# createamind/Distributed-DRL

Hardware: AMD Instinct MI355X
Metric: env-steps/s + learner updates/s, SAC1 LunarLanderContinuous-v2 @1/2/4/8 GPU (higher is better)
Workload: dtype f32

## Files before the change

### distributed-drl_amd/csrc/sac1.hip

```cpp
#include "gemm_core.h"
#include "policy_row.h"

namespace {
struct L1Job {
    const float *in0, *in1, *W, *b;
    float *out, *aug_out;
    int d0, d1, rows, h1, ldo, aug_ld;
    int pre_only;
};
constexpr int MAX_L1_JOBS = 8;
struct OptState;
struct L1Jobs {
    int njobs;
    int noise_on, act, n_each;
    uint32_t noise_seed;
    float *e0, *e1, *e2;
    const OptState *opt;
    L1Job job[MAX_L1_JOBS];
};

constexpr int L1_ROWS = 16;
constexpr int L1_MAXD = 40;
using ddrl_pol::normal_at;
using ddrl_pol::PolRow;
// ... 715 lines not shown
    DDRL_REQUIRE(c->hidden1 <= 64 * RV && c->hidden2 <= 64 * RV, "hidden sizes > 512 unsupported by the row kernels");
    return DDRL_OK;
}

static bool direct_ok(const ddrl_sac1_config_t &c) {
    return c.hidden1 % 4 == 0 && c.hidden2 % 4 == 0 && c.hidden1 <= 512 && c.hidden2 <= 32 * DNT &&
           c.obs_dim + c.act_dim <= 12 && 2 * c.act_dim <= DFH && c.act_dim <= 4 && c.batch <= 4 * DGMAX * 8 &&
           getenv("DDRL_SAC1_GENERIC") == nullptr;
}

}

struct LaunchState {
    int opt_cur;
    int sh_cur;
    bool fuse_apply;
    bool sample_armed;
    bool noise_armed;
    uint32_t noise_seed;
    unsigned int noise_pending;
    bool grad_imported;
};

struct ddrl_sac1 {
    int device;
    ddrl_sac1_config_t cfg;
    Layout L;
    float *slab;
    float *main_p, *target_p, *m, *v, *grad;
    float *in[2][8];
    float *H1, *H2, *dZ2, *dZ1, *xa, *xp, *part;
    float *act0, *act2, *logp0, *logp1, *save0, *q1o, *q2o, *dq4, *dhead, *loss_part, *losses;
    int ldh1, ldh2, ldxa, ldxp, ldd;
    OptState *opt;
    LaunchState ls;
    Seg *segs_d;
    L1Jobs l1a[2];
    GemmJobs g_fa, g_fb, g_bq, g_bpi, g_last;
    RowsA ra[2];
    RowsB rb[2];
    RowsC rc;
    RowsAV rav[2];
    RowsBV rbv[2];
    float *vo, *vto;
    AdamArgs ad;
    int rows_b_blocks;
    bool fused;
    DFHead fh_a[2], fh_b[2];
    DFArgs f_a[2], f_b[2];
    DGJobs dg_bq[2], dg_mid, dg_pi;
    int bq_cols;
    DGJob bq_rest;
    int Lp1, Lp2;
    float *H1r4, *H2c4, *H2r4, *dZ1r4, *dzpi_c4, *dzpi_r4, *dhead_r4, *xa_r4, *da_part, *dq, *w3snap, *xp_r4;
    float *c4_pi[2], *c4_q[3];
    float *c4_q2b;
    int mid_rest_job;
    int bq_q2_job;
    int mid_pi_job, mid_q2w_job;
    int pi_w2_job;
    float *xv_r4;
    int *part_cnt;
    ddrl_replay_dev::RingState *smp_rs;
    ddrl_replay_dev::RingPtrs smp_ring;
    int smp_set;
    float *hp;
    bool fused_l1_wgrad;
    struct HostGraph { const float *block; float *losses; uint32_t seed; int opt_cur, sh_cur; hipGraphExec_t exec; };
    std::vector<HostGraph> host_graphs;
    uint32_t *host_ctr_d;
    struct { bool valid; LaunchState ls; } snap;
};

static void refresh_shadows(ddrl_sac1 *h, hipStream_t s);
int ddrl_internal_normal_fill_ctr(float *out_d, int64_t n, uint32_t seed, const uint32_t *ctr_d, uint64_t base, void *stream);
int ddrl_internal_host_block_up(const float *src, float *dst_d, int64_t n, float *e0, float *e1, float *e2, int64_t m, uint32_t seed,
                                const uint32_t *ctr, void *stream);

static int sac1_free(ddrl_sac1 *h) {
    for (auto &g : h->host_graphs) (void)hipGraphExecDestroy(g.exec);
    if (h->host_ctr_d) (void)hipFree(h->host_ctr_d);
    (void)hipFree(h->slab);
    delete h;
    return DDRL_OK;
}

static int reset_opt(ddrl_sac1 *h, hipStream_t s) {
    OptState o{};
    o.b1p_pi = o.b1p_q = (float)h->cfg.beta1;
    o.b2p_pi = o.b2p_q = (float)h->cfg.beta2;
    h->ls.opt_cur = 0;
    DDRL_HIP_CHECK(hipMemcpyAsync(h->opt, &o, sizeof(o), hipMemcpyHostToDevice, s));
    DDRL_HIP_CHECK(hipStreamSynchronize(s));
    return DDRL_OK;
}

enum { NET_PI = 0, NET_Q1, NET_Q2, NET_V };
enum { ACT_NONE = 0, ACT_STORED, ACT_PI };

struct Eval {
    int net;
    bool x2, targ;
    int act;
    int img = -1;
    bool r4 = false;
    float *ddrl_sac1::*xr4 = nullptr;
    int pev = -1, side = 0;
// ... 216 lines not shown
            dg_add(Q, j);
        }
        for (int q = 0; q < V.nv; ++q) {
            const ValueNet &vn = V.vn[q];
            DGJob j = dq_job(vn.slot, vn.img, q, h->dZ1r4 + q * H1I);
            j.gw_snap = h->w3snap + 512 * q;
            if (vn.net != NET_Q2) { dg_add(Q, j); continue; }
            if (split) j.N = keep * 32;
            h->bq_q2_job = Q.njobs;
            dg_add(Q, j);
            if (split && st == 0) {
                const long long noff = (long long)keep * 32 * 4;
                DGJob r = dq_job(vn.slot, vn.img, q, h->dZ1r4 + q * H1I + noff);
                r.N = h1 - keep * 32;
                r.B = h->c4_q[q] + noff;
                r.mask = h->H1r4 + vn.img * H1I + noff;
                h->bq_rest = r;
            }
        }
    }
    float *G = h->grad;
    const AdamCtx ctx{0, h->main_p, h->target_p, h->m, h->v, G, h->opt, nullptr, L.n_pi_int,
                      (float)cfg->lr, (float)cfg->beta1, (float)cfg->beta2, (float)cfg->adam_eps,
                      (float)cfg->polyak, (float)(1.0 - cfg->polyak), 0u};
    auto wgrad_j4 = [&](const float *A, const float *Bm, long long w_off, long long b_off, float *shadow) {
        DGJob j{};
        j.type = DG_WGRAD_J4; j.M = h1 + 1; j.N = h2; j.K = B;
        j.A = A; j.lda = h->Lp1; j.B = Bm; j.ldb = h->Lp2;
        j.adam_off = w_off; j.ldc = Np2; j.bias_off = b_off; j.bias_row = h1; j.shadow = shadow; j.ld_sh = Kp1;
        return j;
    };
    auto wgrad_rm = [&](const float *A, int lda, int M, const float *Bm, int ldb, int N, long long off) {
        DGJob j{};
        j.type = DG_WGRAD_RM; j.M = M; j.N = N; j.K = B; j.A = A; j.lda = lda; j.B = Bm; j.ldb = ldb; j.adam_off = off; j.ldc = N;
        return j;
    };
    auto head_wgrad = [&](int q) {
        return wgrad_rm(h->H2r4 + V.vn[q].net * H2R, h->Lp2, h2 + 1, h->dq + (long long)q * B, 1, 1, net_off(L, V.vn[q].net).W3);
    };
    {
        DGJobs &M = h->dg_mid;
        M = DGJobs{};
        M.B = B; M.Bv = Bv; M.ad = ctx;
        DGJob d{};
        d.type = DG_DGRAD; d.M = B; d.N = h1; d.K = h2; d.A = h->H2c4; d.lda = B; d.B = h->c4_pi[0]; d.ldb = Kp1;
        d.bgen = 3; d.dap = h->da_part; d.nparts = ct; d.save0 = h->save0; d.wmu = Pm + L.pi_Wmu; d.wls = Pm + L.pi_Wls;
        d.nact = a; d.alpha = (float)cfg->alpha; d.scale = (float)cfg->act_scale;
        d.mask = h->H1r4; d.ldmask = h->Lp1; d.C = h->dZ1r4 + V.nv * H1I; d.ldc = h->Lp1; d.adam_off = -1;
        h->mid_pi_job = M.njobs;
        dg_add(M, d);
        DGJob rc{};
        rc.type = DG_ROWS_C; rc.M = B; rc.N = h2; rc.K = 0; rc.nact = a; rc.adam_off = -1;
        rc.h2c4 = h->H2c4; rc.dap = h->da_part; rc.nparts = ct; rc.save0 = h->save0;
        rc.wmu = Pm + L.pi_Wmu; rc.wls = Pm + L.pi_Wls; rc.dz_c4 = h->dzpi_c4; rc.dz_r4 = h->dzpi_r4; rc.dhead_r4 = h->dhead_r4;
        rc.ld_r4 = h->Lp2; rc.alpha = (float)cfg->alpha; rc.scale = (float)cfg->act_scale;
        dg_add(M, rc);
        for (int q = 0; q < V.nv; ++q) {
            const ValueNet &vn = V.vn[q];
            const NetOff n = net_off(L, vn.net);
            DGJob j = wgrad_j4(h->H1r4 + vn.img * H1I, h->H2r4 + vn.net * H2R, n.W2, n.b2, h->c4_q[q]);
            j.bgen = 1; j.gw = h->w3snap + 512 * q; j.gdq = h->dq + (long long)q * B;
            if (vn.net == NET_Q2) h->mid_q2w_job = M.njobs;
            dg_add(M, j);
        }
        h->mid_rest_job = -1;
        if (!split) {
            for (int q = 0; q < V.nv; ++q) dg_add(M, head_wgrad(q));
        } else {
            const DGJobs &Q0 = h->dg_bq[0];
            M.hp = Q0.hp; M.sacv = 0; M.q_ev0 = Q0.q_ev0; M.q_nev = Q0.q_nev;
            M.b3q1 = Q0.b3q1; M.b3q2 = Q0.b3q2; M.b3q1t = Q0.b3q1t; M.b3q2t = Q0.b3q2t;
            M.rew = Q0.rew; M.done = Q0.done; M.logp0 = Q0.logp0; M.logp1 = Q0.logp1;
            M.q1o = Q0.q1o; M.q2o = Q0.q2o; M.dq = Q0.dq; M.loss_part = Q0.loss_part;
            M.alpha = Q0.alpha; M.gamma = Q0.gamma;
            h->mid_rest_job = M.njobs;
            dg_add(M, h->bq_rest);
        }
    }
    {
        DGJobs &P = h->dg_pi;
        P = DGJobs{};
        P.B = B; P.Bv = Bv; P.ad = ctx;
        h->pi_w2_job = P.njobs;
        dg_add(P, wgrad_j4(h->H1r4, h->dzpi_r4, L.pi_W2, L.pi_b2, h->c4_pi[1]));
        dg_add(P, wgrad_rm(h->H2r4, h->Lp2, h2 + 1, h->dhead_r4, 32, a, L.pi_Wmu));
        dg_add(P, wgrad_rm(h->H2r4, h->Lp2, h2 + 1, h->dhead_r4 + (long long)a * 4, 32, a, L.pi_Wls));
        for (int q = 0; q <= V.nv; ++q) {
            const int net = q < V.nv ? V.vn[q].net : NET_PI;
            const bool xa = net == NET_Q1 || net == NET_Q2;
            DGJob j = wgrad_rm(xa ? h->xa_r4 : (net == NET_V ? h->xv_r4 : h->xp_r4), 32, (xa ? o + a : o) + 1, h->dZ1r4 + q * H1I, h->Lp1, h1, net_off(L, net).W1);
            j.type = DG_WGRAD_W1Y;
            dg_add(P, j);
        }
        if (split)
            for (int q = 0; q < V.nv; ++q) dg_add(P, head_wgrad(q));
        DGJob ls{};
        ls.type = DG_LOSS; ls.M = 1; ls.N = 1; ls.K = 0; ls.adam_off = -1; ls.loss_part = h->loss_part; ls.losses = h->losses; ls.nl = V.nl;
        ls.nparts = -1;
        dg_add(P, ls);
    }
    return DDRL_OK;
}

static void build_rows(ddrl_sac1 *h) {
    const Variant &V = variant_of(h);
    const ddrl_sac1_config_t *cfg = &h->cfg;
    const Layout &L = h->L;
// ... 10 lines not shown
                                (float)cfg->act_scale};
            h->rbv[st] = RowsBV{h->H2, net_q(Pm, L, 0), net_q(Pm, L, 1), net_v(Pm, L), in[3], in[4], h->logp0, h->q1o, h->q2o,
                                h->vo, h->vto, h->dZ2, h->dq4, h->loss_part, B, h2, ldh2, (float)cfg->alpha, (float)cfg->gamma};
        } else {
            h->ra[st] = RowsA{h->H2, net_pi(Pm, L), net_pi(Pt, L), net_q(Pm, L, 0), net_q(Pm, L, 1), in[5], in[6], in[7],
                              h->act0, h->act2, h->logp0, h->logp1, h->save0, h->q1o, h->q2o,
                              h->H1, Pm + L.q_W1[0] + (long long)o * h1, Pt + L.q_W1[0] + (long long)o * h1,
                              Pt + L.q_W1[1] + (long long)o * h1, B, h2, ldh2, a, h1, ldh1, (float)cfg->act_scale};
            h->rb[st] = RowsB{h->H2, net_q(Pm, L, 0), net_q(Pm, L, 1), net_q(Pt, L, 0), net_q(Pt, L, 1), in[3], in[4],
                              h->logp0, h->logp1, h->q1o, h->q2o, h->dZ2, h->dq4, h->loss_part, B, h2, ldh2,
                              (float)cfg->alpha, (float)cfg->gamma};
        }
    }
    h->rc = RowsC{h->H2, at(h->dZ1, 2 * BZ1), Pm + L.q_W1[0], net_pi(Pm, L), h->save0, h->dhead, at(h->dZ2, (V.nv + 1) * BZ2),
                  h->loss_part, h->losses, B, h1, h2, ldh2, o, a, h->ldd, h->rows_b_blocks, (float)cfg->alpha,
                  (float)cfg->act_scale, V.nl};
}

static void init_shape(ddrl_sac1 *h) {
    const ddrl_sac1_config_t &c = h->cfg;
    h->fused = direct_ok(c);
    h->L = make_layout(c, false, h->fused);
    h->Lp1 = rup32(c.hidden1 + 1); h->Lp2 = rup32(c.hidden2 + 1);
    h->ldh1 = (int)pad4(c.hidden1 + 1); h->ldh2 = (int)pad4(c.hidden2 + 1);
    h->ldxa = (int)pad4(c.obs_dim + c.act_dim + 1); h->ldxp = (int)pad4(c.obs_dim + 1); h->ldd = (int)pad4(2 * c.act_dim);
    h->rows_b_blocks = rows_of(h);
    h->mid_rest_job = -1;
}

struct SlabPlan {
    struct Item { float **p; size_t off; };
    std::vector<Item> items;
    size_t floats = 0, cnt_off = 0, opt_off = 0, segs_off = 0;
    size_t reserve(size_t cnt) { const size_t off = floats; floats += (cnt + 63) & ~(size_t)63; return off; }
    void add(float *&p, size_t cnt) { items.push_back(Item{&p, reserve(cnt)}); }
};
static SlabPlan plan_slab(ddrl_sac1 *h) {
    const ddrl_sac1_config_t &c = h->cfg;
    const size_t B = (size_t)rows_of(h), o = c.obs_dim, a = c.act_dim, h1 = c.hidden1, h2 = c.hidden2;
    const size_t NT = (size_t)h->L.total_int, Kp1 = h->L.Kp1, Np2 = h->L.Np2, Lp1 = h->Lp1, Lp2 = h->Lp2;
    SlabPlan p;
    p.add(h->main_p, NT); p.add(h->target_p, NT); p.add(h->m, NT); p.add(h->v, NT); p.add(h->grad, NT);
    for (int st = 0; st < 2; ++st) {
        const size_t cnt[8] = {B * o, B * o, B * a, B, B, B * a, B * a, B * a};
        for (int i = 0; i < 8; ++i) p.add(h->in[st][i], cnt[i]);
    }
    p.add(h->part, ((B + 31) / 32) * (o + 1) * h1);
    if (!h->fused) {
        p.add(h->H1, NEVAL * B * h->ldh1); p.add(h->H2, NEVAL * B * h->ldh2);
        p.add(h->dZ2, 5 * B * h2); p.add(h->dZ1, 5 * B * h1);
    } else {
        const size_t xv = c.variant == DDRL_SAC_V ? 1 : 0;
        p.add(h->H1r4, (4 + xv) * B * Lp1); p.add(h->H2c4, (4 + xv) * Np2 * B); p.add(h->H2r4, (3 + xv) * B * Lp2);
        p.add(h->dZ1r4, (3 + xv) * B * Lp1) ; p.add(h->dzpi_c4, Np2 * B); p.add(h->dzpi_r4, B * Lp2);
        p.add(h->dhead_r4, B * 32); p.add(h->xa_r4, B * 32); p.add(h->xv_r4, B * 32); p.add(h->xp_r4, B * 32); p.add(h->da_part, 16 * B * 4);
        p.add(h->dq, 3 * B + 256); p.add(h->w3snap, 3 * 512);
        for (int i = 0; i < 2; ++i) p.add(h->c4_pi[i], Np2 * Kp1);
        for (size_t i = 0; i < 2 + xv; ++i) p.add(h->c4_q[i], Np2 * Kp1);
        p.add(h->c4_q2b, Np2 * Kp1);
    }
    p.add(h->xa, B * h->ldxa); p.add(h->xp, B * h->ldxp);
    p.add(h->act0, B * a); p.add(h->act2, B * a); p.add(h->logp0, B); p.add(h->logp1, B); p.add(h->save0, B * a * 4);
    p.add(h->q1o, B); p.add(h->q2o, B); p.add(h->vo, B); p.add(h->vto, B); p.add(h->dq4, 3 * B * 4); p.add(h->dhead, B * h->ldd);
    p.add(h->loss_part, (size_t)h->rows_b_blocks * 4); p.add(h->losses, 4);
    p.add(h->hp, (size_t)NEVAL * DFH * B * DNT);
    p.cnt_off = p.reserve(64);
    p.opt_off = p.reserve((2 * sizeof(OptState) + 3) / 4);
    p.segs_off = p.reserve((h->L.segs.size() * sizeof(Seg) + 3) / 4);
    (void)p.reserve(2048);
    return p;
}
static void bind_slab(ddrl_sac1 *h, const SlabPlan &p, float *base) {
    h->slab = base;
    for (const auto &it : p.items) *it.p = base + it.off;
    h->opt = reinterpret_cast<OptState *>(base + p.opt_off);
    h->part_cnt = reinterpret_cast<int *>(base + p.cnt_off);
    h->segs_d = reinterpret_cast<Seg *>(base + p.segs_off);
}
static int alloc_slab(ddrl_sac1 *h, const SlabPlan &p) {
    float *base = nullptr;
    hipError_t e = hipMalloc((void **)&base, p.floats * sizeof(float));
    if (e == hipSuccess) e = hipMemset(base, 0, p.floats * sizeof(float));
    if (e != hipSuccess) {
        ddrl::set_error("hipMalloc of %zu bytes failed in ddrl_sac1_create: %s", p.floats * sizeof(float), hipGetErrorString(e));
        if (base) (void)hipFree(base);
        return DDRL_ERR_NOMEM;
    }
    bind_slab(h, p, base);
    DDRL_HIP_CHECK(hipMemcpy(h->segs_d, h->L.segs.data(), h->L.segs.size() * sizeof(Seg), hipMemcpyHostToDevice));
    return reset_opt(h, nullptr);
}

static int fill_ones(ddrl_sac1 *h) {
    const ddrl_sac1_config_t &c = h->cfg;
    const int B = rows_of(h), o = c.obs_dim, a = c.act_dim, h1 = c.hidden1, h2 = c.hidden2;
    if (!h->fused) {
        k_fill_col<<<(NEVAL * B + 255) / 256, 256>>>(h->H1, (long long)NEVAL * B, h->ldh1, h1, 1.0f);
        k_fill_col<<<(NEVAL * B + 255) / 256, 256>>>(h->H2, (long long)NEVAL * B, h->ldh2, h2, 1.0f);
    } else {
        const int xv = c.variant == DDRL_SAC_V ? 1 : 0;
        k_fill_col4<<<((4 + xv) * B / 4 + 255) / 256, 256>>>(h->H1r4, (long long)(4 + xv) * B / 4, h->Lp1, h1);
        k_fill_col4<<<((3 + xv) * B / 4 + 255) / 256, 256>>>(h->H2r4, (long long)(3 + xv) * B / 4, h->Lp2, h2);
        k_fill_col4<<<(B / 4 + 255) / 256, 256>>>(h->xa_r4, (long long)B / 4, 32, o + a);
        k_fill_col4<<<(B / 4 + 255) / 256, 256>>>(h->xv_r4, (long long)B / 4, 32, o);
        k_fill_col4<<<(B / 4 + 255) / 256, 256>>>(h->xp_r4, (long long)B / 4, 32, o);
    }
    k_fill_col<<<(B + 255) / 256, 256>>>(h->xa, B, h->ldxa, o + a, 1.0f);
// ... 1147 lines not shown
```

### distributed-drl_amd/csrc/sac1_direct.h

```cpp

#ifdef DDRL_STAMPS
static unsigned long long *g_st_host = nullptr;
#define DST(kid, i) do { if (st_ && threadIdx.x == 0) st_[((kid) * 1024 + blockIdx.x) * 16 + (i)] = __builtin_amdgcn_s_memtime(); } while (0)
#define DRT(kid, i) do { if (st_ && threadIdx.x == 0) st_[((kid) * 1024 + blockIdx.x) * 16 + (i)] = __builtin_amdgcn_s_memrealtime(); } while (0)
#else
#define DST(kid, i) do { } while (0)
#define DRT(kid, i) do { } while (0)
#endif

constexpr int DFH = 8;
constexpr int DNT = 16;
constexpr int DGMAX = 16;

__device__ __forceinline__ float f4e(const float4 &v, int e) { return e == 0 ? v.x : (e == 1 ? v.y : (e == 2 ? v.z : v.w)); }

__device__ __forceinline__ void st_img(float *p, const float4 &v) {
    typedef float f4v __attribute__((ext_vector_type(4)));
    f4v t = {v.x, v.y, v.z, v.w};
    __builtin_nontemporal_store(t, reinterpret_cast<f4v *>(p));
}
__device__ __forceinline__ void st_dg(float *p, const float4 &v) {
    typedef float f4v __attribute__((ext_vector_type(4)));
    f4v t = {v.x, v.y, v.z, v.w};
    asm volatile("global_store_dwordx4 %0, %1, off sc1" ::"v"(p), "v"(t) : "memory");
}
__device__ __forceinline__ void st_opt(float *p, const float4 &v) { *reinterpret_cast<float4 *>(p) = v; }
__device__ __forceinline__ int d_slot(int s, int h) { return s < 4 ? 4 * h + s : 8 + 2 * (s - 4) + h; }
__device__ __forceinline__ float relu1(float x) {
    float y;
    asm("v_max_f32 %0, 0, %1" : "=v"(y) : "v"(x));
    return y;
}
static inline int rup32(int x) { return (x + 31) & ~31; }

template <int BYTES>
__device__ __forceinline__ int kline(const void *rec) {
    const int *q = reinterpret_cast<const int *>(rec);
    int acc = q[(BYTES - 4) / 4];
#pragma unroll
    for (int o = 0; o < BYTES - 4; o += 64) acc |= q[o / 4];
    return acc;
}
__device__ __forceinline__ void ktouch(int v) { asm volatile("" ::"s"(v)); }
__device__ __forceinline__ float zero_here() {
    float z = 0.f;
    asm volatile("" : "+v"(z));
    return z;
}

struct DFJob {
    const float *b2;
    const float *wh0, *wh1;
    int nh, hsplit, hstride;
    float *hp;
    float *H2c4;
    float *H2r4;
    float *H1r4;
    float *aug;
    float *xr4;
    int aug_ld;
    const float *php;
    int side;
};
struct DFArgs {
    int njobs, tiles_n, act, Lp1, Lp2, h2;
    float scale;
    float *act0, *act2, *logp0, *logp1, *save0;
    const float *php1;
#ifdef DDRL_STAMPS
    unsigned long long *st;
#endif
    int pev_pack;
    int pin_pack;
    int noise_on, n_each;
    int Bv;
    uint32_t noise_seed;
    float *e0, *e1, *e2;
    const OptState *opt;
    int do_sample, sample_batch;
    ddrl_replay_dev::RingState *rs;
    ddrl_replay_dev::RingPtrs ring;
    ddrl_replay_dev::BatchPtrs sout;
    DFJob job[5];
};
struct DFHead {
    const float *base;
    int tpj, tiles_m;
    int K, Np;
    int B, d0;
    int main_off, targ_off;
    int npi, perq;
    int hp_off;
    int x_off;
    int pack;
};

__host__ __device__ __forceinline__ int pi_bmu_off(int K, int Np, int h2, int act) {
    const int Kp = (K + 31) & ~31;
    return Kp * 16 + Kp * Np + Np + h2 * act;
}
__host__ __device__ __forceinline__ int pi_bls_off(int K, int Np, int h2, int act) { return ((pi_bmu_off(K, Np, h2, act) + act + 3) & ~3) + h2 * act; }

#ifndef DDRL_SIDE_SPREAD
#define DDRL_SIDE_SPREAD 3
#endif
__host__ __device__ __forceinline__ int side_aug_tile(int tiles_n) { return (DDRL_SIDE_SPREAD & 2) ? tiles_n - 1 : 0; }
__host__ __device__ __forceinline__ int side_noise_tile(int tiles_n) { return (DDRL_SIDE_SPREAD & 2) ? (tiles_n > 2 ? tiles_n - 2 : tiles_n - 1) : 0; }
__host__ __device__ __forceinline__ int h1_owned(int b0, int nb, int nt, int tiles_n) {
    if (!(DDRL_SIDE_SPREAD & 1)) return nt == 0 ? 15 : 0;
    int r = b0 % tiles_n, m = 0;
#pragma unroll
    for (int bi = 0; bi < 4; ++bi) {
        if (bi < nb && r == nt) m |= 1 << bi;
        r = r + 1 == tiles_n ? 0 : r + 1;
    }
    return m;
}

template <int NS>
__device__ __forceinline__ void dblock(const float (&w1)[8], const float (&xin)[7], const float4 (&bq)[4], int nrq, floatx16 &x1, floatx16 &acc) {
#pragma unroll
    for (int r = 0; r < 16; ++r) x1[r] = 0.f;
#pragma unroll
    for (int s = 0; s < NS; ++s) x1 = __builtin_amdgcn_mfma_f32_32x32x2f32(w1[s], xin[s], x1, 0, 0, 0);
#pragma unroll
    for (int r = 0; r < 16; ++r) x1[r] = relu1(x1[r]);
#pragma unroll
    for (int rq = 0; rq < 4; ++rq) {
        if (rq < nrq) {
            acc = __builtin_amdgcn_mfma_f32_32x32x2f32(x1[4 * rq + 0], bq[rq].x, acc, 0, 0, 0);
            acc = __builtin_amdgcn_mfma_f32_32x32x2f32(x1[4 * rq + 1], bq[rq].y, acc, 0, 0, 0);
            acc = __builtin_amdgcn_mfma_f32_32x32x2f32(x1[4 * rq + 2], bq[rq].z, acc, 0, 0, 0);
            acc = __builtin_amdgcn_mfma_f32_32x32x2f32(x1[4 * rq + 3], bq[rq].w, acc, 0, 0, 0);
        }
    }
}

struct DOps {
    float4 bq[4][4];
    float w1[4][8];
};
#ifndef DDRL_DPRE0
#define DDRL_DPRE0 1
#endif
#ifndef DDRL_DPRE1
#define DDRL_DPRE1 1
#endif
constexpr int DPRE = 1;
#ifndef DDRL_DGP0
#define DDRL_DGP0 2
#endif
#ifndef DDRL_DGMID
#define DDRL_DGMID 4
#endif
constexpr int DGP0 = DDRL_DGP0;
constexpr int DGMID = DDRL_DGMID;
#ifndef DDRL_DGST
#define DDRL_DGST 5
// ... 208 lines not shown
                ev[c] = pep[0][c];
            }
            const PolRow o = policy_row(mu, ls, ev, d1, a.scale);
    #pragma unroll
            for (int s = 0; s < 7; ++s) {
                const int d = d_slot(s, h), c = d - d0;
                if (d >= d0 && d < D) xin[0][s] = c == 0 ? o.act[0] : (c == 1 ? o.act[1] : (c == 2 ? o.act[2] : o.act[3]));
            }
            if (first_n && w == 0 && lane < 32) {
                const int row = m0 + l31;
                if (jb.side == 1) {
                    a.logp0[row] = o.logp;
    #pragma unroll
                    for (int c = 0; c < 4; ++c)
                        if (c < d1) {
                            a.act0[row * d1 + c] = o.act[c];
                            *reinterpret_cast<float4 *>(a.save0 + ((long long)row * d1 + c) * 4) = make_float4(o.a[c], o.std[c], o.t[c], ev[c]);
                        }
                } else if (jb.side == 2) {
    #pragma unroll
                    for (int c = 0; c < 4; ++c)
                        if (c < d1) a.act2[row * d1 + c] = o.act[c];
                }
            }
            if (two && w == 1) {
    #pragma unroll
                for (int c = 0; c < 4; ++c) {
                    const float o2 = __shfl_xor(hs[1][c], 32);
                    mu[c] = (h ? o2 : hs[1][c]) + pbm[1][c];
                    ls[c] = (h ? hs[1][c] : o2) + pbl[1][c];
                    ev[c] = pep[1][c];
                }
                const PolRow o1 = policy_row(mu, ls, ev, d1, a.scale);
                if (lane < 32) a.logp1[m0 + l31] = o1.logp;
            }
        }
        DST(PH, 2);
        floatx16 acc[MT];
    #pragma unroll
        for (int tt = 0; tt < MT; ++tt)
    #pragma unroll
            for (int r = 0; r < 16; ++r) acc[tt][r] = 0.f;
        float *h1r4 = jb.H1r4;
        const int h1own = h1r4 ? h1_owned(b0, nb, nt, a.tiles_n) : 0;
        {
            if (ns == 4) dkloop<4, MT, PRE>(ops, src, K, lane, xin, acc, h1r4, h1own, a.Lp1, m0, tr[w], epilogue_operands);
            else if (ns == 5) dkloop<5, MT, PRE>(ops, src, K, lane, xin, acc, h1r4, h1own, a.Lp1, m0, tr[w], epilogue_operands);
            else if (ns == 6) dkloop<6, MT, PRE>(ops, src, K, lane, xin, acc, h1r4, h1own, a.Lp1, m0, tr[w], epilogue_operands);
            else dkloop<7, MT, PRE>(ops, src, K, lane, xin, acc, h1r4, h1own, a.Lp1, m0, tr[w], epilogue_operands);
        }

        DST(PH, 3);
        s_wh[tid >> 5][tid & 31] = whv;
        if (nt == side_aug_tile(a.tiles_n) && (jb.aug || jb.xr4)) {
            for (int idx = tid; idx < 32 * MT * D; idx += 256) {
                const int r = idx / D, d = idx - r * D;
                const long long row = m0 + r;
                const float v = d < d0 ? (base + ((jp & 4) ? x2_off : x_off))[row * d0 + d] : (base + a_off)[row * d1 + (d - d0)];
                if (jb.aug) jb.aug[row * jb.aug_ld + d] = v;
                if (jb.xr4) jb.xr4[((row >> 2) * 32 + d) * 4 + (row & 3)] = v;
            }
        }
        if (PH == 0 && a.noise_on && ji == 0 && nt == side_noise_tile(a.tiles_n)) {
            const unsigned long long nbase = a.opt->noise_ctr;
            const int per_row = 3 * act;
            for (int e = tid; e < 32 * MT * per_row; e += 256) {
                const int rr = e / per_row, q = e - rr * per_row;
                const int wch = q / act, c = q - wch * act;
                const int k = (m0 + rr) * act + c;
                if (m0 + rr < a.Bv) (wch == 0 ? a.e0 : (wch == 1 ? a.e1 : a.e2))[k] = normal_at(a.noise_seed, nbase + (unsigned long long)wch * a.n_each + k);
            }
        }

        const int r = tid & 31, cg = tid >> 5;
    #pragma unroll
        for (int tt = 0; tt < MT; ++tt) {
            const int mb = m0 + 32 * tt;
            if (tt > 0) __syncthreads();
    #pragma unroll
            for (int q = 0; q < 16; ++q) red[w][(q & 3) + 8 * (q >> 2) + 4 * h][l31] = acc[tt][q];
            __syncthreads();
            if (tt == 0) DST(PH, 4);
            float v[4];
    #pragma unroll
            for (int e = 0; e < 4; ++e) {
                const int c = 4 * cg + e;
                const float s = ((red[0][r][c] + red[1][r][c]) + red[2][r][c]) + red[3][r][c];
                v[e] = fmaxf(s + (e == 0 ? b4.x : (e == 1 ? b4.y : (e == 2 ? b4.z : b4.w))), 0.f);
            }
            if (jb.H2c4) st_img(jb.H2c4 + ((long long)(n0 / 4 + cg) * B + mb + r) * 4, make_float4(v[0], v[1], v[2], v[3]));
            __syncthreads();
    #pragma unroll
            for (int e = 0; e < 4; ++e) red[0][r][4 * cg + e] = v[e];
            __syncthreads();
            if (jb.H2r4) {
                const int c = tid & 31, rg = tid >> 5;
                if (n0 + c < a.h2)
                    st_img(jb.H2r4 + ((long long)(mb / 4 + rg) * a.Lp2 + n0 + c) * 4,
                           make_float4(red[0][4 * rg][c], red[0][4 * rg + 1][c], red[0][4 * rg + 2][c], red[0][4 * rg + 3][c]));
            }
            {
                const int c = tid >> 5;
                if (c < jb.nh) {
                    float s = 0.f;
    #pragma unroll
                    for (int col = 0; col < 32; ++col) s = fmaf(red[0][r][col], s_wh[c][col], s);
                    jb.hp[((long long)c * B + mb + r) * DNT + nt] = s;
                }
            }
        }
    }
    DST(PH, 5); DRT(PH, 15);
}

// ... 194 lines not shown
                v.w = fmaxf((((p0.w + p1.w) + p2.w) + p3.w) + bb.w, 0.f);
                *reinterpret_cast<float4 *>(&red2[t & 1][r][4 * cg]) = v;
            }
            AST(6 + 5 * t);
            __syncthreads();
            if (cg < 2 * a.act) {
                float sum = 0.f;
#pragma unroll
                for (int c4 = 0; c4 < 8; ++c4) {
                    const float4 x = *reinterpret_cast<const float4 *>(&red2[t & 1][r][4 * c4]), y = *reinterpret_cast<const float4 *>(&s_wh[t][cg][4 * c4]);
                    sum = fmaf(x.x, y.x, sum); sum = fmaf(x.y, y.y, sum); sum = fmaf(x.z, y.z, sum); sum = fmaf(x.w, y.w, sum);
                }
                if (VER) {
                    if (r < vcount) a.hp[((long long)cg * a.rows + a.perm[m0 + r]) * DNT + nt0 + t] = sum;
                } else if (m0 + r < a.rows) a.hp[((long long)cg * a.rows + m0 + r) * DNT + nt0 + t] = sum;
            }
            AST(7 + 5 * t);
        }
    }
}

enum { DG_DGRAD_Q = 0, DG_DGRAD = 1, DG_WGRAD_J4 = 2, DG_WGRAD_RM = 3, DG_ROWS_C = 4, DG_LOSS = 5, DG_WGRAD_W1Y = 6 };
struct alignas(64) DGJob {
    const float *A, *B;
    const float *gp;
    int lda, ldb;
    int K, type;
    int tiles_m, tile_start;
    int slot;
    int bgen;
    int N, ntiles;
    int M;
    const float *gw;
    const float *gdq;
    float *gw_snap;
    float gconst;
    const float *mask;
    int ldmask;
    float *C;
    int ldc;
    const float *wa;
    int wa_d0;
    float *da_part;
    int nact;
    long long adam_off;
    long long bias_off;
    int bias_row;
    float *shadow;
    int ld_sh;
    const float *h2c4;
    const float *dap;
    int nparts;
    const float *save0, *wmu, *wls;
    float *dz_c4, *dz_r4, *dhead_r4;
    int ld_r4;
    float alpha, scale;
    const float *loss_part;
    float *losses;
    int nl;
};
constexpr int MAX_DG_JOBS = 16;
struct DGJobs {
    int njobs, total_tiles;
    int tile_start[MAX_DG_JOBS];
    AdamCtx ad;
    const float *hp;
    const float *b3q1, *b3q2, *b3q1t, *b3q2t;
    const float *rew, *done, *logp0, *logp1;
    float *q1o, *q2o, *dq, *loss_part;
    float *vo, *vto;
#ifdef DDRL_STAMPS
    unsigned long long *st;
#endif
    int sacv;
    int q_ev0, q_nev;
    float alpha, gamma;
    int B, Bv;
    DGJob job[MAX_DG_JOBS];
};


template <int GMAX>
__global__ void __launch_bounds__(256) k_dg(int total_tiles, int tsA, int tsB, int tsC, int tsD, int tsE, int tsF, int tsG, int tsH, int kid, DGJobs jobs) {
    __shared__ __attribute__((aligned(16))) float red[4][32][33];
    __shared__ float s_q[8][32];
    __shared__ float s_g[32];
    __shared__ float s_wa[4][32];
    __shared__ __attribute__((aligned(16))) float s_gw[512];
    __shared__ __attribute__((aligned(16))) float s_w8[512 * 8];
    int t, ji;
#ifdef DDRL_STAMPS
    unsigned long long *const st_ = jobs.st;
#endif
    DRT(kid, 14); DST(kid, 0);
    {
        const int nwg = total_tiles, b = blockIdx.x, q = nwg >> 3, r = nwg & 7, x = b & 7;
        t = (x < r ? x * (q + 1) : r * (q + 1) + (x - r) * q) + (b >> 3);
    }
    static_assert(MAX_DG_JOBS == 16, "k_dg takes tile_start[1..15] as eight scalar arguments, two 16-bit starts each (0xffff: no such job)");
    {
        auto ge2 = [&](int p) { return (t >= (p & 0xffff)) + (t >= (int)((unsigned)p >> 16)); };
        ji = (t >= (int)((unsigned)tsA >> 16)) + ge2(tsB) + ge2(tsC) + ge2(tsD) + ge2(tsE) + ge2(tsF) + ge2(tsG) + ge2(tsH);
    }
    const DGJob &jb = jobs.job[ji];
    typedef int v16i __attribute__((ext_vector_type(16)));
    static_assert(sizeof(DGJob) == 5 * 64 && offsetof(DGJob, M) == 64, "DGJob: hot line = the first 64 bytes, 5 lines in all");
    static_assert(offsetof(DGJobs, job) == 6 * 64, "DGJobs: header of 6 lines, records 64-byte aligned");
    v16i hot;
    int kl;
    {
        constexpr int JOBS_OFF = 64;
        static_assert(alignof(DGJobs) == 64 && 10 * sizeof(int) <= JOBS_OFF, "kernarg offset of k_dg's DGJobs argument");
        const char *ka = (const char *)__builtin_amdgcn_kernarg_segment_ptr();
        const int jboff = __builtin_amdgcn_readfirstlane(JOBS_OFF + (int)offsetof(DGJobs, job) + ji * (int)sizeof(DGJob));
        const void *hdp = ka + JOBS_OFF, *jbp = ka + jboff;
        int k1, k2, k3, k4, k5, k6, k7, k8, k9, k10;
        asm volatile("s_load_dwordx16 %0, %11, 0x0\n\t"
                     "s_load_dword %1, %11, 0x40\n\t"
                     "s_load_dword %2, %11, 0x80\n\t"
                     "s_load_dword %3, %11, 0xc0\n\t"
                     "s_load_dword %4, %11, 0x100\n\t"
                     "s_load_dword %5, %12, 0x0\n\t"
                     "s_load_dword %6, %12, 0x40\n\t"
                     "s_load_dword %7, %12, 0x80\n\t"
                     "s_load_dword %8, %12, 0xc0\n\t"
                     "s_load_dword %9, %12, 0x100\n\t"
                     "s_load_dword %10, %12, 0x140\n\t"
                     "s_waitcnt lgkmcnt(0)"
                     : "=&s"(hot), "=&s"(k1), "=&s"(k2), "=&s"(k3), "=&s"(k4), "=&s"(k5), "=&s"(k6), "=&s"(k7), "=&s"(k8), "=&s"(k9), "=&s"(k10)
                     : "s"(jbp), "s"(hdp)
                     : "memory");
        kl = k1 | k2 | k3 | k4 | k5 | k6 | k7 | k8 | k9 | k10;
    }
    typedef const float __attribute__((address_space(1))) *gfp;
    auto mkptr = [](int lo, int hi) { return (const float *)(gfp)(((unsigned long long)(unsigned)hi << 32) | (unsigned)lo); };
    const float *const hot_A = mkptr(hot[0], hot[1]), *const hot_B = mkptr(hot[2], hot[3]), *const hot_gp = mkptr(hot[4], hot[5]);
    const int hot_lda = hot[6], hot_ldb = hot[7], hot_K = hot[8], hot_type = hot[9], hot_tiles_m = hot[10], hot_tile_start = hot[11];
    const int hot_slot = hot[12], hot_bgen = hot[13], hot_N = hot[14];
    t -= hot_tile_start;
    const int tid = threadIdx.x, lane = tid & 63;
    const int w = __builtin_amdgcn_readfirstlane(tid >> 6);
    const int l31 = lane & 31, h = lane >> 5;
    const int type = hot_type;
    const int Bn = jobs.B, Bv = jobs.Bv;

    if (type == DG_LOSS) {
        if (w != 0) return;
        float s3[4] = {0.f, 0.f, 0.f, 0.f};
        for (int b0 = 0; b0 < Bv; b0 += 64) {
            const int b = b0 + lane;
            const bool ok = b < Bv;
#pragma unroll
            for (int c = 0; c < 4; ++c) {
                const float v = jb.loss_part[(ok ? b : 0) * jb.nl + (c < jb.nl ? c : 0)];
                s3[c] += (ok && c < jb.nl) ? v : 0.f;
            }
        }
#pragma unroll
        for (int c = 0; c < 4; ++c) {
            const float tot = wave_sum(s3[c]);
            const float mean = tot / (float)Bv;
            if (lane == 0 && c < jb.nl) jb.losses[c] = c == 0 ? mean : 0.5f * mean;
        }
        if (lane == 0 && jobs.ad.on && jb.nparts == -1) {
            OptState nx = *jobs.ad.opt;
            nx.b1p_pi *= jobs.ad.b1; nx.b2p_pi *= jobs.ad.b2; nx.b1p_q *= jobs.ad.b1; nx.b2p_q *= jobs.ad.b2;
            nx.t_pi += 1; nx.t_q += 1;
            nx.noise_ctr += jobs.ad.noise_adv;
            *jobs.ad.opt_next = nx;
        }
        return;
    }
    const int tiles_m = hot_tiles_m;
    const int mt = t % tiles_m, nt = t / tiles_m;
    const int m0 = mt * 32, n0 = nt * 32;
    const int r = tid & 31, cg = tid >> 5;

    if (type == DG_ROWS_C) {
        const int act = jb.nact, row = m0 + r;
        float4 dp[16];
#pragma unroll
        for (int q = 0; q < 16; ++q) dp[q] = *reinterpret_cast<const float4 *>(jb.dap + ((long long)(q < jb.nparts ? q : 0) * Bn + row) * 4);
        float4 sv[4];
#pragma unroll
        for (int c = 0; c < 4; ++c) sv[c] = *reinterpret_cast<const float4 *>(jb.save0 + ((long long)row * act + (c < act ? c : 0)) * 4);
        const float4 hm = *reinterpret_cast<const float4 *>(jb.h2c4 + ((long long)(n0 / 4 + cg) * Bn + row) * 4);
        float wm[4][4], wl[4][4];
#pragma unroll
        for (int e = 0; e < 4; ++e) {
            const int c = n0 + 4 * cg + e;
            const bool okc = c < jb.N;
#pragma unroll
            for (int a2 = 0; a2 < 4; ++a2) {
                const long long o = (long long)(okc ? c : 0) * act + (a2 < act ? a2 : 0);
                const float vm = jb.wmu[o], vl = jb.wls[o], keep = (okc && a2 < act) ? 1.0f : 0.f;
                wm[e][a2] = vm * keep;
                wl[e][a2] = vl * keep;
            }
        }
        float ga[4] = {0.f, 0.f, 0.f, 0.f};
#pragma unroll
        for (int q = 0; q < 16; ++q)
            if (q < jb.nparts) { ga[0] += dp[q].x; ga[1] += dp[q].y; ga[2] += dp[q].z; ga[3] += dp[q].w; }
        float dmu[4], dls[4];
#pragma unroll
        for (int c = 0; c < 4; ++c) {
            const float av = sv[c].x, std = sv[c].y, tt = sv[c].z, e = sv[c].w;
            const float glp = row < Bv ? jb.alpha / (float)Bv : 0.f;
            const float om = 1.0f - av * av;
            const float cl = fminf(fmaxf(om, 0.f), 1.f);
            const float du = (ga[c] * jb.scale) * om + glp * ((2.0f * av * om) / (cl + 1e-6f));
            const float sd = std + STD_EPS;
            const float z = (e * std) / sd;
            const float dzdl = ((e * std) * STD_EPS) / (sd * sd);
            const float dl = du * (e * std) + glp * (-(z * dzdl) - 1.0f);
            dmu[c] = c < act ? du : 0.f;
            dls[c] = c < act ? dl * (11.0f * (1.0f - tt * tt)) : 0.f;
        }
        float z4[4];
#pragma unroll
        for (int e = 0; e < 4; ++e) {
            float acc = fmaf(dls[0], wl[e][0], dmu[0] * wm[e][0]);
#pragma unroll
            for (int c = 1; c < 4; ++c) { acc = fmaf(dmu[c], wm[e][c], acc); acc = fmaf(dls[c], wl[e][c], acc); }
            z4[e] = f4e(hm, e) > 0.f ? acc : 0.f;
        }
        st_dg(jb.dz_c4 + ((long long)(n0 / 4 + cg) * Bn + row) * 4, make_float4(z4[0], z4[1], z4[2], z4[3]));
#pragma unroll
        for (int e = 0; e < 4; ++e) red[0][r][4 * cg + e] = z4[e];
        if (nt == 0 && cg == 0) {
#pragma unroll
            for (int c = 0; c < 4; ++c)
                if (c < act) {
                    jb.dhead_r4[((long long)(row >> 2) * 32 + c) * 4 + (row & 3)] = dmu[c];
                    jb.dhead_r4[((long long)(row >> 2) * 32 + act + c) * 4 + (row & 3)] = dls[c];
                }
        }
        __syncthreads();
        {
            const int c = tid & 31, rg = tid >> 5;
            st_dg(jb.dz_r4 + ((long long)(m0 / 4 + rg) * jb.ld_r4 + n0 + c) * 4,
                  make_float4(red[0][4 * rg][c], red[0][4 * rg + 1][c], red[0][4 * rg + 2][c], red[0][4 * rg + 3][c]));
        }
        DST(kid, 5); DRT(kid, 15);
        return;
    }

    const int Kc = hot_K, lda = hot_lda, ldb = hot_ldb;
    const float *Aop = hot_A, *Bop = hot_B;
    const int G = (Kc + 7) >> 3, gs = G >> 2, grem = G & 3;
    const int ng = gs + (w >= 4 - grem ? 1 : 0);
    const int g0 = w * gs + (w > 4 - grem ? w - (4 - grem) : 0);
    const bool first_n = nt == 0;

    const bool need_q = type == DG_DGRAD_Q && hot_slot != 2;
    float4 qv[DNT / 4];
    {
        const int c = tid >> 5;
        const long long HP = (long long)DFH * Bn * DNT;
        const float4 *p4 = reinterpret_cast<const float4 *>(jobs.hp + (jobs.q_ev0 + (c < jobs.q_nev ? c : 0)) * HP + (long long)(m0 + r) * DNT);
#pragma unroll
        for (int q = 0; q < DNT / 4; ++q) qv[q] = make_float4(0.f, 0.f, 0.f, 0.f);
        if (need_q) {
#pragma unroll
            for (int q = 0; q < DNT / 4; ++q) qv[q] = p4[q];
        }
    }
    float rew = 0.f, done = 0.f, lp0 = 0.f, lp1 = 0.f, b3_1 = 0.f, b3_2 = 0.f, b3_1t = 0.f, b3_2t = 0.f;
    if (need_q) {
        if (w == 0) { rew = jobs.rew[m0 + l31]; done = jobs.done[m0 + l31]; lp0 = jobs.logp0[m0 + l31]; lp1 = jobs.logp1[m0 + l31]; }
        b3_1 = jobs.b3q1[0]; b3_2 = jobs.b3q2[0]; b3_1t = jobs.b3q1t[0]; b3_2t = jobs.b3q2t[0];
    }
    const bool has_gen = type == DG_DGRAD_Q || hot_bgen;
    const bool agen = hot_bgen == 3;
    float gv0 = 0.f, gv1 = 0.f, gwn = 0.f;
    if (has_gen) {
        const float *gp = hot_gp;
        const int glen = 8 * G;
        if (hot_bgen != 3) {
            gv0 = gp[tid < glen ? tid : 0];
            gv1 = gp[tid + 256 < glen ? tid + 256 : 0];
            if (type != DG_DGRAD_Q) gwn = jb.gw[(n0 + l31 < hot_N) ? n0 + l31 : 0];
        }
        if (type == DG_DGRAD_Q && jb.gw_snap && t == 0) {
            if (tid < glen) jb.gw_snap[tid] = gv0;
            if (tid + 256 < glen) jb.gw_snap[tid + 256] = gv1;
        }
    }
    float4 a4[GMAX], b4[GMAX];
    const float *Ap = Aop + (long long)(m0 + l31) * 4, *Bp = Bop + (long long)(n0 + l31) * 4;
    const int glast = ng > 0 ? g0 + ng - 1 : (G > 0 ? G - 1 : 0);
    auto fetch_group = [&](int g) {
        const int gg = g0 + g < glast ? g0 + g : glast;
        const long long kg = 2 * gg + h;
        a4[g] = *reinterpret_cast<const float4 *>(Ap + kg * lda * 4);
        b4[g] = *reinterpret_cast<const float4 *>(Bp + kg * ldb * 4);
    };
    constexpr int DGP = DGP0 < GMAX ? DGP0 : GMAX;
    constexpr int DGST = GMAX <= 10 ? DGST10 : GMAX - DGP - 1;
#pragma unroll
    for (int g = 0; g < DGP; ++g) fetch_group(g);
    float pdm[4] = {0.f, 0.f, 0.f, 0.f}, pdl[4] = {0.f, 0.f, 0.f, 0.f};
    if (agen) {
        __builtin_amdgcn_sched_barrier(0);
        const int act = jb.nact, row = m0 + l31;
        float4 dp[16];
#pragma unroll
        for (int q = 0; q < 16; ++q) dp[q] = *reinterpret_cast<const float4 *>(jb.dap + ((long long)(q < jb.nparts ? q : 0) * Bn + row) * 4);
        float4 sv[4];
#pragma unroll
        for (int c = 0; c < 4; ++c) sv[c] = *reinterpret_cast<const float4 *>(jb.save0 + ((long long)row * act + (c < act ? c : 0)) * 4);
        float4 wm4[2], wl4[2];
        const int k0 = tid, k1 = tid + 256;
        const bool ok0 = k0 < Kc, ok1 = k1 < Kc;
        const long long kb0 = (long long)(ok0 ? k0 : 0) * act, kb1 = (long long)(ok1 ? k1 : 0) * act;
        if (act == 2) {
            const float2 a0 = *reinterpret_cast<const float2 *>(jb.wmu + kb0), b0 = *reinterpret_cast<const float2 *>(jb.wls + kb0);
            const float2 a1 = *reinterpret_cast<const float2 *>(jb.wmu + kb1), b1 = *reinterpret_cast<const float2 *>(jb.wls + kb1);
            const float e0 = ok0 ? 1.0f : 0.f, e1 = ok1 ? 1.0f : 0.f;
            wm4[0] = make_float4(a0.x * e0, a0.y * e0, 0.f, 0.f); wl4[0] = make_float4(b0.x * e0, b0.y * e0, 0.f, 0.f);
            wm4[1] = make_float4(a1.x * e1, a1.y * e1, 0.f, 0.f); wl4[1] = make_float4(b1.x * e1, b1.y * e1, 0.f, 0.f);
        } else {
            float am[2][4], al[2][4];
#pragma unroll
            for (int a2 = 0; a2 < 4; ++a2) {
                const int ao = a2 < act ? a2 : 0;
                am[0][a2] = jb.wmu[kb0 + ao]; al[0][a2] = jb.wls[kb0 + ao]; am[1][a2] = jb.wmu[kb1 + ao]; al[1][a2] = jb.wls[kb1 + ao];
            }
#pragma unroll
            for (int a2 = 0; a2 < 4; ++a2) {
                const float e0 = (ok0 && a2 < act) ? 1.0f : 0.f, e1 = (ok1 && a2 < act) ? 1.0f : 0.f;
                am[0][a2] *= e0; al[0][a2] *= e0; am[1][a2] *= e1; al[1][a2] *= e1;
            }
            wm4[0] = make_float4(am[0][0], am[0][1], am[0][2], am[0][3]); wl4[0] = make_float4(al[0][0], al[0][1], al[0][2], al[0][3]);
            wm4[1] = make_float4(am[1][0], am[1][1], am[1][2], am[1][3]); wl4[1] = make_float4(al[1][0], al[1][1], al[1][2], al[1][3]);
        }
        DST(kid, 6);
        float ga[4] = {0.f, 0.f, 0.f, 0.f};
#pragma unroll
        for (int q = 0; q < 16; ++q)
            if (q < jb.nparts) { ga[0] += dp[q].x; ga[1] += dp[q].y; ga[2] += dp[q].z; ga[3] += dp[q].w; }
#pragma unroll
        for (int c = 0; c < 4; ++c) {
            const float av = sv[c].x, std = sv[c].y, tt = sv[c].z, e = sv[c].w;
            const float glp = row < Bv ? jb.alpha / (float)Bv : 0.f;
            const float om = 1.0f - av * av;
            const float cl = fminf(fmaxf(om, 0.f), 1.f);
            const float du = (ga[c] * jb.scale) * om + glp * ((2.0f * av * om) / (cl + 1e-6f));
            const float sd = std + STD_EPS;
            const float z = (e * std) / sd;
            const float dzdl = ((e * std) * STD_EPS) / (sd * sd);
            const float dl = du * (e * std) + glp * (-(z * dzdl) - 1.0f);
            pdm[c] = c < act ? du : 0.f;
            pdl[c] = c < act ? dl * (11.0f * (1.0f - tt * tt)) : 0.f;
        }
        DST(kid, 7);
#pragma unroll
        for (int u = 0; u < 2; ++u) {
            const int k = tid + 256 * u;
            if (k < 8 * G) {
                if (act <= 2) *reinterpret_cast<float4 *>(&s_w8[k * 4]) = make_float4(wm4[u].x, wm4[u].y, wl4[u].x, wl4[u].y);
                else { *reinterpret_cast<float4 *>(&s_w8[k * 8]) = wm4[u]; *reinterpret_cast<float4 *>(&s_w8[k * 8 + 4]) = wl4[u]; }
            }
        }
        DST(kid, 8);
    }
    const bool agen2 = agen && jb.nact <= 2;
    ktouch(kl);
    DST(kid, 1);
    const bool is_dgrad = type == DG_DGRAD_Q || type == DG_DGRAD;
    float4 mk = make_float4(1.f, 1.f, 1.f, 1.f);
    float wa_v = 0.f;
    const bool has_da = is_dgrad && jb.da_part;
    const bool rm_like = type == DG_WGRAD_RM || type == DG_WGRAD_W1Y;
    const bool do_adam = jobs.ad.on && (type == DG_WGRAD_J4 || rm_like) && jb.adam_off >= 0;
    const bool narrow = rm_like && hot_N <= 8;
    float al_pi = 0.f, al_q = 0.f;
    float b1p_pi = 0.f, b2p_pi = 0.f, b1p_q = 0.f, b2p_q = 0.f;
    float4 j_m, j_v, j_p, j_t;
    float bm = 0.f, bv = 0.f, bp = 0.f, bt = 0.f;
    float am[4], av[4], ap[4], at[4];
    bool okv[4];
    long long j_idx = 0, b_idx = 0;
    bool j_ok = false, b_ok = false;
    auto epilogue_operands = [&](auto kind) {
        constexpr int KIND = decltype(kind)::value;
        if (KIND == 0) {
            if (is_dgrad) mk = *reinterpret_cast<const float4 *>(jb.mask + ((long long)(m0 / 4 + cg) * jb.ldmask + n0 + r) * 4);
            if (has_da) {
                const int c = tid >> 5, col = n0 + (tid & 31);
// ... 315 lines not shown
```

Baseline: 47580.

## Trim redundant global loads and stores in SAC backward row kernels

Removes the unused dz_c4 output buffer and its store, and drops the unused aug copy path. The side-tile xr4 image is now written from registers already holding the inputs rather than re-read from global memory. In the DG_ROWS_C and agen paths, each half-wave loads only half of the dap partials and save0 entries, and a permlane32 swap rebuilds the full set, roughly halving redundant load requests. For act==2 it also loads the weights as float2. The gains rely on the permlane swap's lane mapping matching the half index, which adds correctness risk.

```diff
diff --git a/distributed-drl_amd/csrc/sac1.hip b/distributed-drl_amd/csrc/sac1.hip
--- a/distributed-drl_amd/csrc/sac1.hip
+++ b/distributed-drl_amd/csrc/sac1.hip
@@ -791,7 +791,7 @@
     int bq_cols;
     DGJob bq_rest;
     int Lp1, Lp2;
-    float *H1r4, *H2c4, *H2r4, *dZ1r4, *dzpi_c4, *dzpi_r4, *dhead_r4, *xa_r4, *da_part, *dq, *w3snap, *xp_r4;
+    float *H1r4, *H2c4, *H2r4, *dZ1r4, *dzpi_r4, *dhead_r4, *xa_r4, *da_part, *dq, *w3snap, *xp_r4;
     float *c4_pi[2], *c4_q[3];
     float *c4_q2b;
     int mid_rest_job;
@@ -1114,7 +1114,7 @@
         DGJob rc{};
         rc.type = DG_ROWS_C; rc.M = B; rc.N = h2; rc.K = 0; rc.nact = a; rc.adam_off = -1;
         rc.h2c4 = h->H2c4; rc.dap = h->da_part; rc.nparts = ct; rc.save0 = h->save0;
-        rc.wmu = Pm + L.pi_Wmu; rc.wls = Pm + L.pi_Wls; rc.dz_c4 = h->dzpi_c4; rc.dz_r4 = h->dzpi_r4; rc.dhead_r4 = h->dhead_r4;
+        rc.wmu = Pm + L.pi_Wmu; rc.wls = Pm + L.pi_Wls; rc.dz_r4 = h->dzpi_r4; rc.dhead_r4 = h->dhead_r4;
         rc.ld_r4 = h->Lp2; rc.alpha = (float)cfg->alpha; rc.scale = (float)cfg->act_scale;
         dg_add(M, rc);
         for (int q = 0; q < V.nv; ++q) {
@@ -1231,7 +1231,7 @@
     } else {
         const size_t xv = c.variant == DDRL_SAC_V ? 1 : 0;
         p.add(h->H1r4, (4 + xv) * B * Lp1); p.add(h->H2c4, (4 + xv) * Np2 * B); p.add(h->H2r4, (3 + xv) * B * Lp2);
-        p.add(h->dZ1r4, (3 + xv) * B * Lp1) ; p.add(h->dzpi_c4, Np2 * B); p.add(h->dzpi_r4, B * Lp2);
+        p.add(h->dZ1r4, (3 + xv) * B * Lp1) ; p.add(h->dzpi_r4, B * Lp2);
         p.add(h->dhead_r4, B * 32); p.add(h->xa_r4, B * 32); p.add(h->xv_r4, B * 32); p.add(h->xp_r4, B * 32); p.add(h->da_part, 16 * B * 4);
         p.add(h->dq, 3 * B + 256); p.add(h->w3snap, 3 * 512);
         for (int i = 0; i < 2; ++i) p.add(h->c4_pi[i], Np2 * Kp1);
diff --git a/distributed-drl_amd/csrc/sac1_direct.h b/distributed-drl_amd/csrc/sac1_direct.h
--- a/distributed-drl_amd/csrc/sac1_direct.h
+++ b/distributed-drl_amd/csrc/sac1_direct.h
@@ -56,9 +56,7 @@
     float *H2c4;
     float *H2r4;
     float *H1r4;
-    float *aug;
     float *xr4;
-    int aug_ld;
     const float *php;
     int side;
 };
@@ -104,6 +102,9 @@
 #ifndef DDRL_SIDE_SPREAD
 #define DDRL_SIDE_SPREAD 3
 #endif
+#ifndef DDRL_REQ_DIET
+#define DDRL_REQ_DIET 19
+#endif
 __host__ __device__ __forceinline__ int side_aug_tile(int tiles_n) { return (DDRL_SIDE_SPREAD & 2) ? tiles_n - 1 : 0; }
 __host__ __device__ __forceinline__ int side_noise_tile(int tiles_n) { return (DDRL_SIDE_SPREAD & 2) ? (tiles_n > 2 ? tiles_n - 2 : tiles_n - 1) : 0; }
 __host__ __device__ __forceinline__ int h1_owned(int b0, int nb, int nt, int tiles_n) {
@@ -418,14 +419,27 @@
 
         DST(PH, 3);
         s_wh[tid >> 5][tid & 31] = whv;
-        if (nt == side_aug_tile(a.tiles_n) && (jb.aug || jb.xr4)) {
+        if (nt == side_aug_tile(a.tiles_n) && jb.xr4) {
+#if DDRL_REQ_DIET & 16
+            if (w == 0) {
+#pragma unroll
+                for (int tt = 0; tt < MT; ++tt) {
+                    const long long row = m0 + 32 * tt + l31;
+#pragma unroll
+                    for (int s = 0; s < 7; ++s) {
+                        const int d = d_slot(s, h);
+                        if (d < D) jb.xr4[((row >> 2) * 32 + d) * 4 + (row & 3)] = xin[tt][s];
+                    }
+                }
+            }
+#else
             for (int idx = tid; idx < 32 * MT * D; idx += 256) {
                 const int r = idx / D, d = idx - r * D;
                 const long long row = m0 + r;
                 const float v = d < d0 ? (base + ((jp & 4) ? x2_off : x_off))[row * d0 + d] : (base + a_off)[row * d1 + (d - d0)];
-                if (jb.aug) jb.aug[row * jb.aug_ld + d] = v;
-                if (jb.xr4) jb.xr4[((row >> 2) * 32 + d) * 4 + (row & 3)] = v;
-            }
+                jb.xr4[((row >> 2) * 32 + d) * 4 + (row & 3)] = v;
+            }
+#endif
         }
         if (PH == 0 && a.noise_on && ji == 0 && nt == side_noise_tile(a.tiles_n)) {
             const unsigned long long nbase = a.opt->noise_ctr;
@@ -726,7 +740,7 @@
     const float *dap;
     int nparts;
     const float *save0, *wmu, *wls;
-    float *dz_c4, *dz_r4, *dhead_r4;
+    float *dz_r4, *dhead_r4;
     int ld_r4;
     float alpha, scale;
     const float *loss_part;
@@ -753,6 +767,16 @@
     DGJob job[MAX_DG_JOBS];
 };
 
+
+__device__ __forceinline__ void row_pairs(const float4 &v, float4 &ev, float4 &od) {
+    typedef unsigned u2v __attribute__((ext_vector_type(2)));
+    const u2v x = __builtin_amdgcn_permlane32_swap(__float_as_uint(v.x), __float_as_uint(v.x), false, false);
+    const u2v y = __builtin_amdgcn_permlane32_swap(__float_as_uint(v.y), __float_as_uint(v.y), false, false);
+    const u2v z = __builtin_amdgcn_permlane32_swap(__float_as_uint(v.z), __float_as_uint(v.z), false, false);
+    const u2v w = __builtin_amdgcn_permlane32_swap(__float_as_uint(v.w), __float_as_uint(v.w), false, false);
+    ev = make_float4(__uint_as_float(x[0]), __uint_as_float(y[0]), __uint_as_float(z[0]), __uint_as_float(w[0]));
+    od = make_float4(__uint_as_float(x[1]), __uint_as_float(y[1]), __uint_as_float(z[1]), __uint_as_float(w[1]));
+}
 
 template <int GMAX>
 __global__ void __launch_bounds__(256) k_dg(int total_tiles, int tsA, int tsB, int tsC, int tsD, int tsE, int tsF, int tsG, int tsH, int kid, DGJobs jobs) {
@@ -852,14 +876,39 @@
 
     if (type == DG_ROWS_C) {
         const int act = jb.nact, row = m0 + r;
-        float4 dp[16];
-#pragma unroll
-        for (int q = 0; q < 16; ++q) dp[q] = *reinterpret_cast<const float4 *>(jb.dap + ((long long)(q < jb.nparts ? q : 0) * Bn + row) * 4);
+        constexpr bool HSPLIT = (DDRL_REQ_DIET & 1) != 0;
+        float4 dp[16], dph[8], svh[2];
         float4 sv[4];
-#pragma unroll
-        for (int c = 0; c < 4; ++c) sv[c] = *reinterpret_cast<const float4 *>(jb.save0 + ((long long)row * act + (c < act ? c : 0)) * 4);
+        if (HSPLIT) {
+#pragma unroll
+            for (int i = 0; i < 8; ++i) dph[i] = *reinterpret_cast<const float4 *>(jb.dap + ((long long)(2 * i + h < jb.nparts ? 2 * i + h : 0) * Bn + row) * 4);
+            svh[0] = *reinterpret_cast<const float4 *>(jb.save0 + ((long long)row * act + (h < act ? h : 0)) * 4);
+            svh[1] = svh[0];
+        } else {
+#pragma unroll
+            for (int q = 0; q < 16; ++q) dp[q] = *reinterpret_cast<const float4 *>(jb.dap + ((long long)(q < jb.nparts ? q : 0) * Bn + row) * 4);
+#pragma unroll
+            for (int c = 0; c < 4; ++c) sv[c] = *reinterpret_cast<const float4 *>(jb.save0 + ((long long)row * act + (c < act ? c : 0)) * 4);
+        }
         const float4 hm = *reinterpret_cast<const float4 *>(jb.h2c4 + ((long long)(n0 / 4 + cg) * Bn + row) * 4);
         float wm[4][4], wl[4][4];
+        if ((DDRL_REQ_DIET & 2) && act == 2) {
+            float2 m2[4], l2[4];
+#pragma unroll
+            for (int e = 0; e < 4; ++e) {
+                const int c = n0 + 4 * cg + e;
+                const long long o = (long long)(c < jb.N ? c : 0) * 2;
+                m2[e] = *reinterpret_cast<const float2 *>(jb.wmu + o);
+                l2[e] = *reinterpret_cast<const float2 *>(jb.wls + o);
+            }
+#pragma unroll
+            for (int e = 0; e < 4; ++e) {
+                const float keep = n0 + 4 * cg + e < jb.N ? 1.0f : 0.f;
+                wm[e][0] = m2[e].x * keep; wm[e][1] = m2[e].y * keep; wm[e][2] = m2[e].x * 0.f; wm[e][3] = m2[e].x * 0.f;
+                wl[e][0] = l2[e].x * keep; wl[e][1] = l2[e].y * keep; wl[e][2] = l2[e].x * 0.f; wl[e][3] = l2[e].x * 0.f;
+            }
+        } else {
+        if (HSPLIT) svh[1] = *reinterpret_cast<const float4 *>(jb.save0 + ((long long)row * act + (2 + h < act ? 2 + h : 0)) * 4);
 #pragma unroll
         for (int e = 0; e < 4; ++e) {
             const int c = n0 + 4 * cg + e;
@@ -871,6 +920,13 @@
                 wm[e][a2] = vm * keep;
                 wl[e][a2] = vl * keep;
             }
+        }
+        }
+        if (HSPLIT) {
+#pragma unroll
+            for (int i = 0; i < 8; ++i) row_pairs(dph[i], dp[2 * i], dp[2 * i + 1]);
+            row_pairs(svh[0], sv[0], sv[1]);
+            row_pairs(svh[1], sv[2], sv[3]);
         }
         float ga[4] = {0.f, 0.f, 0.f, 0.f};
 #pragma unroll
@@ -899,7 +955,6 @@
             for (int c = 1; c < 4; ++c) { acc = fmaf(dmu[c], wm[e][c], acc); acc = fmaf(dls[c], wl[e][c], acc); }
             z4[e] = f4e(hm, e) > 0.f ? acc : 0.f;
         }
-        st_dg(jb.dz_c4 + ((long long)(n0 / 4 + cg) * Bn + row) * 4, make_float4(z4[0], z4[1], z4[2], z4[3]));
 #pragma unroll
         for (int e = 0; e < 4; ++e) red[0][r][4 * cg + e] = z4[e];
         if (nt == 0 && cg == 0) {
@@ -978,12 +1033,20 @@
     if (agen) {
         __builtin_amdgcn_sched_barrier(0);
         const int act = jb.nact, row = m0 + l31;
-        float4 dp[16];
-#pragma unroll
-        for (int q = 0; q < 16; ++q) dp[q] = *reinterpret_cast<const float4 *>(jb.dap + ((long long)(q < jb.nparts ? q : 0) * Bn + row) * 4);
+        constexpr bool HSPLIT = (DDRL_REQ_DIET & 1) != 0;
+        float4 dp[16], dph[8], svh[2];
         float4 sv[4];
-#pragma unroll
-        for (int c = 0; c < 4; ++c) sv[c] = *reinterpret_cast<const float4 *>(jb.save0 + ((long long)row * act + (c < act ? c : 0)) * 4);
+        if (HSPLIT) {
+#pragma unroll
+            for (int i = 0; i < 8; ++i) dph[i] = *reinterpret_cast<const float4 *>(jb.dap + ((long long)(2 * i + h < jb.nparts ? 2 * i + h : 0) * Bn + row) * 4);
+            svh[0] = *reinterpret_cast<const float4 *>(jb.save0 + ((long long)row * act + (h < act ? h : 0)) * 4);
+            svh[1] = svh[0];
+        } else {
+#pragma unroll
+            for (int q = 0; q < 16; ++q) dp[q] = *reinterpret_cast<const float4 *>(jb.dap + ((long long)(q < jb.nparts ? q : 0) * Bn + row) * 4);
+#pragma unroll
+            for (int c = 0; c < 4; ++c) sv[c] = *reinterpret_cast<const float4 *>(jb.save0 + ((long long)row * act + (c < act ? c : 0)) * 4);
+        }
         float4 wm4[2], wl4[2];
         const int k0 = tid, k1 = tid + 256;
         const bool ok0 = k0 < Kc, ok1 = k1 < Kc;
@@ -995,6 +1058,7 @@
             wm4[0] = make_float4(a0.x * e0, a0.y * e0, 0.f, 0.f); wl4[0] = make_float4(b0.x * e0, b0.y * e0, 0.f, 0.f);
             wm4[1] = make_float4(a1.x * e1, a1.y * e1, 0.f, 0.f); wl4[1] = make_float4(b1.x * e1, b1.y * e1, 0.f, 0.f);
         } else {
+            if (HSPLIT) svh[1] = *reinterpret_cast<const float4 *>(jb.save0 + ((long long)row * act + (2 + h < act ? 2 + h : 0)) * 4);
             float am[2][4], al[2][4];
 #pragma unroll
             for (int a2 = 0; a2 < 4; ++a2) {
@@ -1010,6 +1074,12 @@
             wm4[1] = make_float4(am[1][0], am[1][1], am[1][2], am[1][3]); wl4[1] = make_float4(al[1][0], al[1][1], al[1][2], al[1][3]);
         }
         DST(kid, 6);
+        if (HSPLIT) {
+#pragma unroll
+            for (int i = 0; i < 8; ++i) row_pairs(dph[i], dp[2 * i], dp[2 * i + 1]);
+            row_pairs(svh[0], sv[0], sv[1]);
+            row_pairs(svh[1], sv[2], sv[3]);
+        }
         float ga[4] = {0.f, 0.f, 0.f, 0.f};
 #pragma unroll
         for (int q = 0; q < 16; ++q)
```

Result: no change. 47610 (median of 3 runs) (+0.1%).
